# songrise/HyperNeRF-torch

Hardware: AMD Instinct MI355X
Metric: ray-samples/sec (fwd+bwd+Adam), whole job; per-GPU = value/n_gpus (higher is better)
Workload: dtype bf16; 1 GPU; NerfModel use_warp bendy_sheet nerf_embed+alpha_cond, 1024 rays x (64+64) samples per GPU, fwd+bwd+Adam; rays_per_gpu=1024, n_samples=64, n_importance=64, parallelism=dp1, hip_graph=True, wgrad_schedule=serial: one batched launch, optimizer_launch=hn_adam_step, ranks_seen_by_collective=1

## Files before the change

hypernerf-torch_amd/_lib.py:

```python
from __future__ import annotations

import ctypes as C
import os
import subprocess

import numpy as np
import torch

_HERE = os.path.dirname(os.path.abspath(__file__))
CSRC = os.path.join(_HERE, "csrc")
PRODUCT_LIB_PATH = os.path.join(CSRC, "libhn_hip.so")
LIB_PATH = os.environ.get("HN_LIB_PATH") or PRODUCT_LIB_PATH
SOURCES = ["hn_mlp.hip", "hn_render.hip", "hn_calib.hip", "hn_optim.hip"]
CSRC_HEADERS = ["hn_common.h", "hn_pack.h"]
HEADER = os.path.join(os.path.dirname(_HERE), "include", "hn_kernels.h")
BUILD_MACROS = ("HN_REDUCE_SPLIT", "HN_BF16_WAVES", "HN_PROF", "HN_CHUNK_UNITS", "HN_WGRAD_AUX", "HN_WGRAD_STAGES", "HN_WGRAD_MAXSLOT")

HN_MODE_F32, HN_MODE_BF16, HN_MODE_BF16_S8 = 0, 1, 2
BUILD_CONFIG_KEYS = ("WGRAD_STAGES", "WGRAD_MAXSLOT", "WGRAD_BIAS_MFMA", "CHUNK_UNITS", "WGRAD_BLOCK", "WSTREAM_ASYM",
                     "BF16_WAVES", "WGRAD_AUX")


def _read_build_config(path: str):
    import re
    try:
        with open(path, "rb") as f:
            blob = f.read()
    except OSError:
        return None
    m = re.search(rb"HN_BUILD_CONFIG:([0-9, ]+);", blob)
    if m is None:
        return None
    vals = [int(x) for x in m.group(1).decode().replace(" ", "").split(",")]
    return {k: v for k, v in zip(BUILD_CONFIG_KEYS, vals)}


BUILD_CONFIG = _read_build_config(LIB_PATH)
_cfg = BUILD_CONFIG or {}
WGRAD_STAGES = _cfg.get("WGRAD_STAGES", int(os.environ.get("HN_WGRAD_STAGES") or 2))
WGRAD_MAXSLOT = _cfg.get("WGRAD_MAXSLOT", int(os.environ.get("HN_WGRAD_MAXSLOT") or 8))
WGRAD_MAX_STAGE_KB = min(8 * WGRAD_MAXSLOT, 160 // WGRAD_STAGES)
HN_MAX_SRC, HN_MAX_DST, HN_MAX_SLOTS = 8, 4, 128
HN_OP_WORDS, HN_CHUNK_UNITS, HN_DSRC_COMPS = 8, _cfg.get("CHUNK_UNITS", int(os.environ.get("HN_CHUNK_UNITS", 32))), 32
HN_AUXG_MAX = 3
HN_MAX_COMPS = 32

HN_OP_LAYER, HN_OP_OUT, HN_OP_OUT_WIDE = 1, 4, 5
HN_ACT_NONE, HN_ACT_RELU, HN_ACT_LEAKY_RELU, HN_ACT_ELU, HN_ACT_SOFTPLUS = 0, 1, 2, 3, 4
HN_LAYER_NO_COMMIT, HN_LAYER_DIRECT = 1, 2
HN_BOP_LOAD, HN_BOP_LOAD_WIDE, HN_BOP_LAYER, HN_BOP_AUX = 1, 2, 3, 4
HN_FEAT_ZERO, HN_FEAT_ID, HN_FEAT_SIN, HN_FEAT_COS, HN_FEAT_SINP, HN_FEAT_ID_DIRECT = 0, 1, 2, 3, 4, 5


class HnSrc(C.Structure):
    _fields_ = [("ptr", C.c_void_p), ("ld", C.c_int32), ("per_ray", C.c_int32), ("gather_idx", C.c_void_p),
                ("gather_rows", C.c_int32), ("pad", C.c_int32)]


class HnDst(C.Structure):
    _fields_ = [("ptr", C.c_void_p), ("ld", C.c_int32), ("pad", C.c_int32)]


class HnSlot(C.Structure):
    _fields_ = [("off", C.c_uint64), ("nt", C.c_int32), ("pad", C.c_int32)]


class HnMlpArgs(C.Structure):
    _fields_ = [
        ("mode", C.c_int32), ("n_points", C.c_int32), ("samples_per_ray", C.c_int32), ("training", C.c_int32),
        ("n_ops", C.c_int32), ("n_chunks", C.c_int32), ("n_dsrc", C.c_int32), ("n_bias", C.c_int32),
        ("n_feat", C.c_int32), ("max_groups", C.c_int32),
        ("ops", C.c_void_p), ("wstream", C.c_void_p), ("bias", C.c_void_p), ("feat", C.c_void_p),
        ("stash", C.c_void_p), ("masks", C.c_void_p), ("dsrc", C.c_void_p),
        ("src", HnSrc * HN_MAX_SRC), ("dst", HnDst * HN_MAX_DST), ("slots", HnSlot * HN_MAX_SLOTS),
        ("prof", C.c_void_p), ("comps", C.c_void_p), ("n_comps", C.c_int32), ("embed_reg_mask", C.c_int32),
        ("embed_grad", C.c_void_p), ("embed_idx", C.c_void_p), ("embed_rows", C.c_int32), ("embed_dim", C.c_int32),
        ("embed_col", C.c_int8 * 32), ("n_trig_comps", C.c_int32), ("wide_ops", C.c_int32), ("dz_scale_log2", C.c_int32), ("trig_lo_planes", C.c_int32),
        ("timeline", C.c_void_p), ("embed_partial", C.c_void_p),
    ]


class HnDwBatch(C.Structure):
    _fields_ = [("jobs", C.c_void_p), ("stash", C.c_void_p), ("grads", C.c_void_p), ("n_jobs", C.c_int32),
                ("pad", C.c_int32), ("partials", C.c_void_p)]


HN_MAX_WGRAD_BATCH = 8
HN_MAX_DRAWS = 8


HN_MAX_PACK_JOBS = 8


class HnPackJob(C.Structure):
    _fields_ = [("units", C.c_void_p), ("ptrs", C.c_void_p), ("wstream", C.c_void_p), ("bias", C.c_void_p),
                ("bias_out", C.c_void_p), ("n_units", C.c_int32), ("n_bias", C.c_int32)]


class HnEmbedReduce(C.Structure):
    _fields_ = [("grad", C.c_void_p), ("rows", C.c_int32), ("dim", C.c_int32), ("col_mask", C.c_uint32), ("n_src", C.c_int32),
                ("partial", C.c_void_p * HN_MAX_WGRAD_BATCH), ("idx", C.c_void_p * HN_MAX_WGRAD_BATCH),
                ("n_blocks", C.c_int32 * HN_MAX_WGRAD_BATCH), ("samples_per_ray", C.c_int32 * HN_MAX_WGRAD_BATCH)]


class HnDraw(C.Structure):
    _fields_ = [("ptr", C.c_void_p), ("n", C.c_int64), ("kind", C.c_int32), ("pad", C.c_int32)]


class HnPrologue(C.Structure):
    _fields_ = [("t_rand_draw", C.c_int32), ("n_rays", C.c_int32), ("n", C.c_int32), ("ray_ld", C.c_int32),
                ("per_ray_bounds", C.c_int32), ("scale", C.c_float),
                ("origins", C.c_void_p), ("dirs", C.c_void_p), ("lower", C.c_void_p), ("upper", C.c_void_p),
                ("z_out", C.c_void_p), ("pts_out", C.c_void_p), ("ids_src", C.c_void_p), ("ids_dst", C.c_void_p),
                ("ids_ld", C.c_int32), ("n_ids", C.c_int32)]


class HnCompositeArgs(C.Structure):
    _fields_ = [
        ("variant", C.c_int32), ("n_rays", C.c_int32), ("n_samples", C.c_int32), ("white_bg", C.c_int32),
        ("sample_at_infinity", C.c_int32), ("warped_ld", C.c_int32), ("has_dust", C.c_int32), ("dust_threshold", C.c_float),
        ("rgb", C.c_void_p), ("raw", C.c_void_p), ("noise", C.c_void_p), ("z", C.c_void_p), ("dirs", C.c_void_p),
        ("ray_ld", C.c_int64), ("warped", C.c_void_p),
        ("out_rgb", C.c_void_p), ("out_depth", C.c_void_p), ("out_acc", C.c_void_p), ("out_weights", C.c_void_p),
        ("out_med_depth", C.c_void_p), ("out_med_points", C.c_void_p),
        ("g_rgb", C.c_void_p), ("g_depth", C.c_void_p), ("g_acc", C.c_void_p), ("g_weights", C.c_void_p),
        ("d_rgb", C.c_void_p), ("d_raw", C.c_void_p), ("keep", C.c_void_p),
        ("noise_scale", C.c_float), ("split", C.c_int32),
        ("perm", C.c_void_p), ("rgb1", C.c_void_p), ("raw1", C.c_void_p), ("warped1", C.c_void_p),
        ("d_rgb1", C.c_void_p), ("d_raw1", C.c_void_p), ("out_warped", C.c_void_p),
    ]


PACK_UNIT_DT = np.dtype([("w_id", "<i4"), ("ld", "<i4"), ("r0", "<i4"), ("c0", "<i4"), ("r_end", "<i4"),
                         ("c_end", "<i4"), ("k0", "<i4"), ("transposed", "<i4")])
PACK_BIAS_DT = np.dtype([("w_id", "<i4"), ("n", "<i4"), ("off", "<i4"), ("len", "<i4")])
FEAT_DT = np.dtype([("packed", "<i4"), ("freq", "<f4")])
DWJOB_DT = np.dtype([("z_off", "<u8"), ("x_off", "<u8"), ("z_nt", "<i4"), ("x_nt", "<i4"), ("z_t0", "<i4"),
                     ("x_t0", "<i4"), ("n_nt", "<i4"), ("n_kt", "<i4"), ("blk0", "<i4"), ("blk1", "<i4"),
                     ("w_off", "<i4"), ("ld", "<i4"), ("r0", "<i4"), ("c0", "<i4"), ("r_end", "<i4"),
                     ("c_end", "<i4"), ("b_off", "<i4"), ("pad", "<i4"), ("x2_off", "<u8"), ("x2_nt", "<i4"),
                     ("x2_t0", "<i4"), ("n_kt1", "<i4"), ("p_tile", "<i4")])
DWREDUCE_DT = np.dtype([("batch", "<i4"), ("w_off", "<i4"), ("ld", "<i4"), ("row0", "<i4"), ("col0", "<i4"),
                        ("r_end", "<i4"), ("c_end", "<i4"), ("first", "<i4"), ("count", "<i4")])

ADAM_RANGE_DT = np.dtype([("start", "<i8"), ("len", "<i4"), ("pad", "<i4")])


class HnAdamFuse(C.Structure):
    _fields_ = [("params", C.c_void_p), ("grads", C.c_void_p), ("exp_avg", C.c_void_p), ("exp_avg_sq", C.c_void_p),
                ("n", C.c_int64), ("hyper", C.c_void_p), ("step", C.c_void_p), ("rest", C.c_void_p),
                ("n_rest", C.c_int32), ("zero_grad", C.c_int32)]


EXPORTS = ["hn_version", "hn_abi_sizes", "hn_build_config", "hn_mlp_wgrad_reduce_adam", "hn_render_prologue", "hn_pack_units", "hn_pack_units_multi", "hn_mlp_forward", "hn_mlp_backward", "hn_mlp_wgrad",
           "hn_mlp_wgrad_batched", "hn_mlp_wgrad_batched_t", "hn_mlp_wgrad_reduce", "hn_mlp_workspace_bytes",
           "hn_sample_along_rays", "hn_sample_legacy", "hn_posenc", "hn_composite_forward", "hn_composite_backward", "hn_sample_pdf", "hn_sample_pdf_split", "hn_composite_sample_pdf",
           "hn_embed_gather", "hn_embed_backward", "hn_se3_apply_forward", "hn_se3_apply_backward", "hn_se3_warp_forward", "hn_se3_warp_backward", "hn_generate_rays", "hn_adam_step", "hn_sgd_step", "hn_radam_step",
           "hn_mse_loss_forward", "hn_mse_loss_backward", "hn_mse_loss_forward_grad", "hn_depth_index", "hn_random_fill",
           "hn_probe_mfma", "hn_calib_mfma", "hn_calib_stream", "hn_calib_stream_pattern", "hn_calib_ring"]

_lib = None


class HnError(RuntimeError):
    pass


def hipcc_path() -> str:
    for cand in (os.environ.get("HIPCC"), "/opt/rocm/bin/hipcc", "hipcc"):
        if cand and (os.path.isabs(cand) and os.path.exists(cand) or not os.path.isabs(cand)):
            return cand
    return "hipcc"


def needs_build() -> bool:
    if not os.path.exists(PRODUCT_LIB_PATH):
        return True
    t = os.path.getmtime(PRODUCT_LIB_PATH)
    deps = [os.path.join(CSRC, s) for s in SOURCES] + [os.path.join(CSRC, h) for h in CSRC_HEADERS] + [HEADER]
    return any(os.path.getmtime(d) > t for d in deps)


def build(force: bool = False, verbose: bool = False) -> str:
    if not force and not needs_build():
        return PRODUCT_LIB_PATH
    out = os.environ.get("HN_BUILD_OUT") or PRODUCT_LIB_PATH
    cmd = [hipcc_path(), "--offload-arch=gfx950", "-O3", "-std=c++17", "-ffp-contract=off", "-munsafe-fp-atomics", "-fPIC", "-shared",
           "-o", out] + [os.path.join(CSRC, s) for s in SOURCES]
    for macro in BUILD_MACROS:
        if os.environ.get(macro):
            cmd.insert(1, f"-D{macro}={os.environ[macro]}")
    res = subprocess.run(cmd, capture_output=True, text=True)
    if res.returncode != 0:
        raise HnError("hipcc failed:\n" + " ".join(cmd) + "\n" + res.stdout + res.stderr)
    if verbose:
        print(res.stdout + res.stderr)
    return out


def build_id() -> dict:
    import hashlib
    h = hashlib.sha256()
    for d in [os.path.join(CSRC, s) for s in SOURCES] + [os.path.join(CSRC, h) for h in CSRC_HEADERS] + [HEADER]:
        with open(d, "rb") as f:
            h.update(f.read())
    for macro in BUILD_MACROS:
        h.update(f"{macro}={os.environ.get(macro, '')};".encode())
    lib = None
    if os.path.exists(LIB_PATH):
        with open(LIB_PATH, "rb") as f:
            lib = hashlib.sha256(f.read()).hexdigest()[:16]
    ident = {"kernel_src_sha256": h.hexdigest()[:16], "lib_sha256": lib}
    if LIB_PATH != PRODUCT_LIB_PATH:
        ident["lib_path_override"] = LIB_PATH
        ident["kernel_src_sha256"] = "override:" + (lib or "?")
    if BUILD_CONFIG is not None:
        ident["build_config"] = dict(BUILD_CONFIG)
    return ident


def load():
    global _lib
    if _lib is not None:
        return _lib
    if not os.path.exists(LIB_PATH):
        raise HnError(
            f"{LIB_PATH} is missing: the HIP extension has not been built (run __graft_entry__.build()). "
            "hypernerf_torch_amd has no CPU fallback.")
    lib = C.CDLL(LIB_PATH)
    for name in EXPORTS:
        if not hasattr(lib, name):
            raise HnError(f"{LIB_PATH} does not export {name}")
        getattr(lib, name).restype = C.c_int
    buf = (C.c_int32 * len(BUILD_CONFIG_KEYS))()
    n_cfg = lib.hn_build_config(buf, len(BUILD_CONFIG_KEYS))
    now = {k: int(buf[i]) for i, k in enumerate(BUILD_CONFIG_KEYS[:n_cfg])}
    mine = {"WGRAD_STAGES": WGRAD_STAGES, "WGRAD_MAXSLOT": WGRAD_MAXSLOT, "CHUNK_UNITS": HN_CHUNK_UNITS}
    bad = {k: (v, now.get(k)) for k, v in mine.items() if now.get(k) != v}
    if bad:
        raise HnError(f"{LIB_PATH} was built with other tuning knobs than the host tables assume (mirror, library): {bad}; "
                      "re-import hypernerf_torch_amd after building, or unset the HN_* build variables")
    _lib = lib
    return lib


KERNEL_TIMES = None
_PENDING = []
PROF_BUFFER = None


def launch(name: str, *args, tag: str = ""):
    fn = getattr(load(), name)
    if KERNEL_TIMES is None:
        check(fn(*args), name + (f"[{tag}]" if tag else ""))
        return
    e0, e1 = torch.cuda.Event(enable_timing=True), torch.cuda.Event(enable_timing=True)
    e0.record()
    rc = fn(*args)
    e1.record()
    _PENDING.append((name + (f"[{tag}]" if tag else ""), e0, e1))
    check(rc, name)


TIMELINE = None
TIMELINE_TICK_S = 1e-8


def timeline_slot(name: str, device) -> int:
    if TIMELINE is None:
        return 0
    t = TIMELINE.get(name)
    if t is None:
        if torch.cuda.is_current_stream_capturing():
            raise HnError(f"kernel timeline: first launch of {name} inside a stream capture (run a warm-up step first)")
        t = TIMELINE[name] = torch.zeros(8, dtype=torch.int64, device=device)
    return t.data_ptr()


def timeline_reset():
    torch.cuda.synchronize()
    for t in (TIMELINE or {}).values():
        t.zero_()
    torch.cuda.synchronize()


def timeline_read() -> dict:
    torch.cuda.synchronize()
    out = {}
    for name, t in (TIMELINE or {}).items():
        v = t.cpu().tolist()
        out[name] = {"ms": v[4] * TIMELINE_TICK_S * 1e3, "runs": int(v[5]), "span_ms": (v[7] - v[6]) * TIMELINE_TICK_S * 1e3,
                     "first_start_tick": v[6], "last_end_tick": v[7]}
    return out


def collect_kernel_times():
    torch.cuda.synchronize()
    for name, e0, e1 in _PENDING:
        KERNEL_TIMES.setdefault(name, []).append(e0.elapsed_time(e1))
    _PENDING.clear()
    return KERNEL_TIMES


def check(rc: int, what: str):
    if rc != 0:
        kind = "argument error" if rc < 0 else "hipError_t"
        raise HnError(f"{what} failed: {kind} {rc}")


def stream_handle() -> C.c_void_p:
    return C.c_void_p(torch.cuda.current_stream().cuda_stream)


def require_gpu(*tensors):
    for t in tensors:
        if t is not None and not t.is_cuda:
            raise HnError("hypernerf_torch_amd runs on MI355X only: got a CPU tensor and there is no CPU fallback "
                          "(the CPU oracle lives in oracle/ and is test infrastructure)")

# ... 14 lines not shown
```

hypernerf-torch_amd/csrc/hn_mlp.hip:

```cpp
#include "hn_common.h"
#include <algorithm>
#include <type_traits>

#ifdef HN_PROF
#define HN_STAMP(code)                                                                          \
  do {                                                                                          \
    if (prof_on && prof_n < 2040) {                                                             \
      unsigned long long t__;                                                                   \
      __builtin_amdgcn_sched_barrier(0);                                                        \
      asm volatile("s_memtime %0\n\ts_waitcnt lgkmcnt(0)" : "=s"(t__)::"memory");               \
      __builtin_amdgcn_sched_barrier(0);                                                        \
      if (lane == 0) { prof_buf[2 * prof_n] = (code); prof_buf[2 * prof_n + 1] = (long long)t__; } \
      ++prof_n;                                                                                 \
    }                                                                                           \
  } while (0)
#else
#define HN_STAMP(code) do {} while (0)
#endif

template <int WAVES>
struct WStream {
  const char* g;
  char* lds;
  int ctr;
// ... 131 lines not shown
    va[j] = *reinterpret_cast<const float*>(srcv_r + (t[j][0] & 0xffffu));
    vb[j] = *reinterpret_cast<const float*>(srcv_r + (t[j][0] >> 16));
  }
  __builtin_amdgcn_sched_barrier(0);
#pragma unroll
  for (int j = 0; j < 4; ++j) {
    const float f = __uint_as_float(t[j][1]);
    const float big = __builtin_amdgcn_fractf(__fmul_rn(f, va[j]));
    const float sv = __builtin_amdgcn_sinf(__fadd_rn(big, __builtin_fmaf(f, vb[j], __uint_as_float(t[j][2]))));
    out[j] = hn_bfi(t[j][3], va[j], sv);
  }
}
HN_DEV void hn_feature_grads4(const HnDFeat* tp, const char* srcv_r, float* out) {
  u32x4 t[4];
#pragma unroll
  for (int j = 0; j < 4; ++j) t[j] = reinterpret_cast<const u32x4*>(tp)[j];
  __builtin_amdgcn_sched_barrier(0);
  float x[4];
#pragma unroll
  for (int j = 0; j < 4; ++j) x[j] = *reinterpret_cast<const float*>(srcv_r + t[j][0]);
  __builtin_amdgcn_sched_barrier(0);
#pragma unroll
  for (int j = 0; j < 4; ++j) {
    const float sc = __uint_as_float(t[j][1]);
    const float g = (sc * 6.283185307179586f) * hn_sin_rev(__builtin_fmaf(sc, x[j], __uint_as_float(t[j][2]) + 0.25f));
    out[j] = hn_bfi(t[j][3], 1.0f, g);
  }
}

template <bool BF16, bool DIRECT>
HN_DEV float hn_feature(const HnFeat e, const float* srcv, int r, const HnMlpArgs& a, int p, int ray) {
  const int kind = (e.packed >> 12) & 15;
  if constexpr (DIRECT) {
    if (kind == HN_FEAT_ID_DIRECT) return hn_direct_source(e, a, p, ray);
  }
  const float x = srcv[(e.packed & 255) * 32 + r];
  if constexpr (BF16) {
    const float ph = (kind == HN_FEAT_COS || kind == HN_FEAT_SINP) ? 0.25f : 0.0f;
    const float s = hn_sin_rev(__builtin_fmaf(e.freq * HN_INV_2PI, x, ph));
    return kind == HN_FEAT_ID ? x : (kind == HN_FEAT_ZERO ? 0.0f : s);
  } else {
    if (kind == HN_FEAT_ZERO) return 0.0f;
    if (kind == HN_FEAT_ID) return x;
    float arg = __fmul_rn(e.freq, x);
    if (kind == HN_FEAT_SINP) arg = __fadd_rn(arg, 0.5f * 3.1415926f);
    return kind == HN_FEAT_COS ? cosf(arg) : sinf(arg);
  }
}

template <bool BF16>
HN_DEV float hn_feature_grad(const HnFeat e, const float* srcv, int r) {
  const int kind = (e.packed >> 12) & 15;
  const float x = srcv[(e.packed & 255) * 32 + r];
  if constexpr (BF16) {
    const float ph = (kind == HN_FEAT_COS || kind == HN_FEAT_SINP) ? 0.5f : 0.25f;
    const float g = e.freq * hn_sin_rev(__builtin_fmaf(e.freq * HN_INV_2PI, x, ph));
    return (kind == HN_FEAT_ID || kind == HN_FEAT_ID_DIRECT) ? 1.0f : g;
  } else {
    if (kind == HN_FEAT_ID || kind == HN_FEAT_ID_DIRECT) return 1.0f;
    float arg = __fmul_rn(e.freq, x);
    if (kind == HN_FEAT_SINP) arg = __fadd_rn(arg, 0.5f * 3.1415926f);
    if (kind == HN_FEAT_COS) return -e.freq * sinf(arg);
    return e.freq * cosf(arg);
  }
}

template <bool DIRECT>
HN_DEV void hn_make_group(bf16x8* out, const HnFeat* ft, const HnDFeat* dft, const float* srcv, int lane,
                          const HnMlpArgs& a, int p, int ray) {
  const int h = lane >> 5, r = lane & 31;
  if constexpr (DIRECT) {
#pragma unroll
    for (int s = 0; s < 4; ++s) {
#pragma unroll
      for (int j = 0; j < 8; ++j)
        out[s][j] = (__bf16)hn_feature<true, true>(ft[16 * s + hn_pi16(h, j)], srcv, r, a, p, ray);
    }
  } else {
    const char* srcv_r = reinterpret_cast<const char*>(srcv) + 4 * r;
#pragma unroll
    for (int s = 0; s < 4; ++s) {
      float v[8];
      hn_features4(dft + 16 * s + 4 * h, srcv_r, v);
      hn_features4(dft + 16 * s + 8 + 4 * h, srcv_r, v + 4);
#pragma unroll
      for (int j = 0; j < 8; ++j) out[s][j] = (__bf16)v[j];
    }
  }
}
template <bool DIRECT>
HN_DEV void hn_make_group(float* out, const HnFeat* ft, const HnDFeat*, const float* srcv, int lane, const HnMlpArgs& a,
                          int p, int ray) {
  const int h = lane >> 5, r = lane & 31;
#pragma unroll
  for (int s = 0; s < 32; ++s) {
    out[s] = hn_feature<false, DIRECT>(ft[32 * (s >> 4) + hn_rho(s & 15, h)], srcv, r, a, p, ray);
    if ((s & 7) == 7) __builtin_amdgcn_sched_barrier(0);
  }
}

HN_DEV void hn_init_acc(f32x16& acc, const float* bias, int t, int h) {
  if (bias != nullptr) {
#pragma unroll
    for (int g = 0; g < 4; ++g) {
      const f32x4 b = *reinterpret_cast<const f32x4*>(bias + 32 * t + 8 * g + 4 * h);
      acc[4 * g] = b[0]; acc[4 * g + 1] = b[1]; acc[4 * g + 2] = b[2]; acc[4 * g + 3] = b[3];
    }
  } else {
#pragma unroll
    for (int i = 0; i < 16; ++i) acc[i] = 0.0f;
  }
}

constexpr int HN_PF = 3;
template <bool BF16, int K32>
HN_DEV void hn_gemm_blocks(f32x16& acc, const typename ModeT<BF16>::Frag* in, WStream<ModeT<BF16>::WAVES>& ws) {
  using M = ModeT<BF16>;
  const char* w = ws.take(K32 * M::UNITS32);
  if constexpr (BF16) {
    constexpr int N = 2 * K32;
    constexpr int D = N < HN_PF ? N : HN_PF;
    const char* wl = w + ws.lane * 16;
    bf16x8 q[D];
#pragma unroll
    for (int u = 0; u < D; ++u) q[u] = *reinterpret_cast<const bf16x8*>(wl + u * 1024);
#pragma unroll
    for (int u = 0; u < N; ++u) {
      acc = hn_mfma_bf16(q[u % D], in[u], acc);
      if (u + D < N) q[u % D] = *reinterpret_cast<const bf16x8*>(wl + (u + D) * 1024);
    }
    __builtin_amdgcn_sched_group_barrier(0x100, D, 0);
#pragma unroll
    for (int u = 0; u < N; ++u) {
      __builtin_amdgcn_sched_group_barrier(0x008, 1, 0);
      if (u + D < N) __builtin_amdgcn_sched_group_barrier(0x100, 1, 0);
    }
  } else {
#pragma unroll
    for (int k = 0; k < K32; ++k) hn_mma_block32(acc, w + k * M::UNITS32 * 1024, in + k * M::STEPS32, ws.lane);
  }
}
template <bool BF16>
HN_DEV void hn_gemm_k(f32x16& acc, const typename ModeT<BF16>::Frag* in, int K32, WStream<ModeT<BF16>::WAVES>& ws) {
  if (K32 == 8) hn_gemm_blocks<BF16, 8>(acc, in, ws);
  else if (K32 == 4) hn_gemm_blocks<BF16, 4>(acc, in, ws);
  else if (K32 == 2) hn_gemm_blocks<BF16, 2>(acc, in, ws);
  else if (K32 == 1) hn_gemm_blocks<BF16, 1>(acc, in, ws);
}

template <bool BF16, int S8 = 0>
HN_DEV char* hn_slot_base(const HnMlpArgs& a, int off_kib, int nt, int blk) {
  if (off_kib < 0) return nullptr;
  constexpr int TU = S8 ? 1 : ModeT<BF16>::TILE_UNITS;
  return reinterpret_cast<char*>(a.stash) + (size_t)(unsigned)off_kib * 1024 + (size_t)blk * nt * (TU * 1024);
}
HN_DEV uint32_t* hn_mask_base(const HnMlpArgs& a, int off256, int nt, int blk, int lane) {
  (void)lane;
  return a.masks + (size_t)(unsigned)off256 * 64 + (size_t)blk * nt * 64;
}
HN_DEV int hn_stash_slot(int r, int h, int u) { return 32 * h + (r ^ (4 * h + 8 * u)); }
HN_DEV int hn_stash8_slot(int r, int h) { return (r & 3) + 4 * h + 8 * ((r >> 2) & 1) + 16 * (r >> 3); }
template <int S8>
HN_DEV int hn_cvt2_f8(unsigned w, int old, bool hi) {
  const float lo_f = __uint_as_float(w << 16), hi_f = __uint_as_float(w & 0xffff0000u);
  if constexpr (S8 == 1) return hi ? __builtin_amdgcn_cvt_pk_fp8_f32(lo_f, hi_f, old, true)
                                   : __builtin_amdgcn_cvt_pk_fp8_f32(lo_f, hi_f, old, false);
  else return hi ? __builtin_amdgcn_cvt_pk_bf8_f32(lo_f, hi_f, old, true)
                 : __builtin_amdgcn_cvt_pk_bf8_f32(lo_f, hi_f, old, false);
}
template <int S8>
HN_DEV void hn_stash8_acc(const f32x16& a, char* slot_base, int t, int lane) {
  u32x4 o;
#pragma unroll
  for (int k = 0; k < 4; ++k) {
    int w = 0;
    if constexpr (S8 == 1) {
      w = __builtin_amdgcn_cvt_pk_fp8_f32(a[4 * k], a[4 * k + 1], w, false);
      w = __builtin_amdgcn_cvt_pk_fp8_f32(a[4 * k + 2], a[4 * k + 3], w, true);
    } else {
      w = __builtin_amdgcn_cvt_pk_bf8_f32(a[4 * k], a[4 * k + 1], w, false);
      w = __builtin_amdgcn_cvt_pk_bf8_f32(a[4 * k + 2], a[4 * k + 3], w, true);
    }
    o[k] = (unsigned)w;
  }
  char* dst8 = slot_base + (size_t)t * 1024 + hn_stash8_slot(lane & 31, lane >> 5) * 16;
  __builtin_nontemporal_store(o, reinterpret_cast<u32x4*>(dst8));
}
template <bool BF16, int S8 = 0>
HN_DEV void hn_stash(const typename ModeT<BF16>::Frag* fr, char* slot_base, int t, int lane) {
  using M = ModeT<BF16>;
  if constexpr (BF16 && S8 != 0) {
    const u32x4 f0 = *reinterpret_cast<const u32x4*>(&fr[0]), f1 = *reinterpret_cast<const u32x4*>(&fr[1]);
    u32x4 o;
#pragma unroll
    for (int k = 0; k < 2; ++k) {
      int lo = 0, hi = 0;
      lo = hn_cvt2_f8<S8>(f0[2 * k], lo, false);
      lo = hn_cvt2_f8<S8>(f0[2 * k + 1], lo, true);
      hi = hn_cvt2_f8<S8>(f1[2 * k], hi, false);
      hi = hn_cvt2_f8<S8>(f1[2 * k + 1], hi, true);
      o[k] = (unsigned)lo;
      o[2 + k] = (unsigned)hi;
    }
    char* dst8 = slot_base + (size_t)t * 1024 + hn_stash8_slot(lane & 31, lane >> 5) * 16;
    __builtin_nontemporal_store(o, reinterpret_cast<u32x4*>(dst8));
    return;
  }
  char* dst = slot_base + (size_t)t * (M::TILE_UNITS * 1024);
  if constexpr (BF16) {
    const int off0 = hn_stash_slot(lane & 31, lane >> 5, 0) * 16;
    __builtin_nontemporal_store(*reinterpret_cast<const u32x4*>(&fr[0]), reinterpret_cast<u32x4*>(dst + off0));
    __builtin_nontemporal_store(*reinterpret_cast<const u32x4*>(&fr[1]), reinterpret_cast<u32x4*>(dst + 1024 + (off0 ^ 128)));
  } else {
    const f32x16 z = hn_transpose_tile(fr, lane);
    hn_store_tile(z, dst, lane, (typename M::Frag*)nullptr);
  }
}

template <bool BF16>
HN_DEV unsigned hn_push_mask(unsigned bits, float x) {
  if constexpr (BF16) return __builtin_amdgcn_alignbit(bits, __float_as_uint(x), 31);
  return (bits << 1) | (x > 0.0f ? 0u : 1u);
}
HN_DEV int hn_keep_mask(unsigned nbits, int q, int i) { return (int)(nbits << (16 * q + i)) >> 31; }

template <bool BF16>
HN_DEV void hn_act_tile(f32x16& acc, int act, float p0, float p1, unsigned& bits) {
  if (act == HN_ACT_LEAKY_RELU) {
#pragma unroll 1
    for (int i = 0; i < 16; ++i) {
      bits = hn_push_mask<false>(bits, acc[i]);
      acc[i] = acc[i] > 0.0f ? acc[i] : p0 * acc[i];
    }
  } else if (act == HN_ACT_ELU) {
#pragma unroll 1
    for (int i = 0; i < 16; ++i) {
      const float z = acc[i];
      const float em1 = BF16 ? __expf(z) - 1.0f : expm1f(z);
      acc[i] = z > 0.0f ? z : p0 * em1;
    }
  } else if (act == HN_ACT_SOFTPLUS) {
    const float inv = 1.0f / p0;
#pragma unroll 1
    for (int i = 0; i < 16; ++i) {
      const float z = acc[i], u = z * p0;
      const float sp = BF16 ? __logf(1.0f + __expf(u)) : log1pf(expf(u));
      acc[i] = u > p1 ? z : (BF16 ? sp * inv : sp / p0);
    }
  }
}
template <bool BF16>
HN_DEV float hn_dact_y(int act, float y, float p0, float p1) {
  if (act == HN_ACT_ELU) return y > 0.0f ? 1.0f : y + p0;
  const float u = p0 * y;
  return u > p1 ? 1.0f : (BF16 ? 1.0f - __expf(-u) : -expm1f(-u));
}
template <bool BF16>
HN_DEV f32x16 hn_unstash(const char* slot_base, int t, int lane) {
  using M = ModeT<BF16>;
  const char* src = slot_base + (size_t)t * (M::TILE_UNITS * 1024);
  f32x16 y;
  if constexpr (BF16) {
    const int off0 = hn_stash_slot(lane & 31, lane >> 5, 0) * 16;
    const u32x4 f0 = *reinterpret_cast<const u32x4*>(src + off0);
    const u32x4 f1 = *reinterpret_cast<const u32x4*>(src + 1024 + (off0 ^ 128));
#pragma unroll
    for (int k = 0; k < 4; ++k) {
      y[2 * k] = __uint_as_float(f0[k] << 16);
      y[2 * k + 1] = __uint_as_float(f0[k] & 0xffff0000u);
      y[8 + 2 * k] = __uint_as_float(f1[k] << 16);
      y[8 + 2 * k + 1] = __uint_as_float(f1[k] & 0xffff0000u);
    }
  } else {
    float z[16];
#pragma unroll
    for (int g = 0; g < 4; ++g) {
      const f32x4 v = *reinterpret_cast<const f32x4*>(src + g * 1024 + lane * 16);
#pragma unroll
      for (int e = 0; e < 4; ++e) z[4 * g + e] = v[e];
    }
    y = hn_transpose_tile(z, lane);
  }
  return y;
}

typedef const __attribute__((address_space(4))) int* HnOpPtr;
HN_DEV HnOpPtr hn_op_words(const int* ops, int op) {
  return (HnOpPtr)(uintptr_t)(ops + (size_t)op * HN_OP_WORDS);
}
struct HnOpWords {
  int v[HN_OP_WORDS];
  HN_DEV int operator[](int i) const { return v[i]; }
};
HN_DEV HnOpWords hn_load_op(const int* ops, int op, int n_ops) {
  HnOpWords w;
  const HnOpPtr p = hn_op_words(ops, op < n_ops ? op : n_ops - 1);
#pragma unroll
  for (int i = 0; i < HN_OP_WORDS; ++i) w.v[i] = p[i];
  if (op >= n_ops) w.v[0] = -1;
  return w;
}


template <bool TRAIN, int NT, int S8>
HN_DEV void hn_epilogue_share(int k, int tp, f32x16& a, bf16x8* frag, unsigned& bits, char* out_base,
                              uint32_t* mask_base, int lane) {
  if (k < 8) {
#pragma unroll
    for (int e = 0; e < 2; ++e) {
      const int i = 2 * k + e;
      if (TRAIN) bits = hn_push_mask<true>(bits, a[i]);
      frag[i >> 3][i & 7] = (__bf16)__int_as_float(max(__float_as_int(a[i]), 0));
    }
  } else if (TRAIN && k == 8) {
    hn_stash<true, S8>(frag, out_base, tp, lane);
    if ((tp & 1) || tp == NT - 1) {
      mask_base[(tp >> 1) * 64 + lane] = (tp & 1) ? bits : bits << 16;
      bits = 0;
    }
  }
}

template <int K32, int NT, bool TRAIN, int S8>
HN_DEV void hn_layer_pipelined(bf16x8* cur, bf16x8* nxt, const float* bias, WStream<ModeT<true>::WAVES>& ws,
                               char* out_base, uint32_t* mask_base, int lane) {
  constexpr int N = 2 * K32;
  constexpr int D = 2;
  constexpr int SHARES = 9;
  constexpr int PER_SLOT = (SHARES + N - 1) / N;
  const int h = lane >> 5;
  f32x16 acc[2];
  unsigned bits = 0;
#pragma unroll
  for (int t = 0; t <= NT; ++t) {
    const char* wl = nullptr;
    if (t < NT) wl = ws.take(N) + lane * 16;
    const int tp = t - 1;
    bf16x8 q[D];
    if (t < NT) {
      hn_init_acc(acc[t & 1], bias, t, h);
#pragma unroll
      for (int u = 0; u < D; ++u) q[u] = *reinterpret_cast<const bf16x8*>(wl + u * 1024);
    }
    __builtin_amdgcn_sched_barrier(0);
#pragma unroll
    for (int u = 0; u < N; ++u) {
      if (t < NT) {
        acc[t & 1] = hn_mfma_bf16(q[u % D], cur[u], acc[t & 1]);
        if (u + D < N) q[u % D] = *reinterpret_cast<const bf16x8*>(wl + (u + D) * 1024);
      }
      if (t > 0) {
#pragma unroll
        for (int e = 0; e < PER_SLOT; ++e) {
          const int k = u * PER_SLOT + e;
          if (k < SHARES)
            hn_epilogue_share<TRAIN, NT, S8>(k, tp, acc[tp & 1], nxt + tp * 2, bits, out_base, mask_base, lane);
        }
      }
      __builtin_amdgcn_sched_barrier(0);
    }
  }
#pragma unroll
  for (int i = 0; i < NT * 2; ++i) cur[i] = nxt[i];
}

template <bool BF16, int AUXG, bool EXTRA, bool TRAIN, bool S8 = false>
__global__ __launch_bounds__(ModeT<BF16>::WAVES * 64, BF16 ? 2 : 1) void hn_mlp_fwd_kernel(const HnMlpArgs a) {
  using M = ModeT<BF16>;
  constexpr int SX = S8 ? 1 : 0;
  static_assert(!(S8 && (EXTRA || !TRAIN || !BF16)), "the 8-bit stash exists for the render-level bf16 training builds only");
  if constexpr (S8) asm volatile("s_setreg_imm32_b32 hwreg(HW_REG_MODE, 23, 1), 1");
  using Frag = typename M::Frag;
  extern __shared__ __attribute__((aligned(16))) char smem[];
  const int lane = threadIdx.x & 63;
  const int wave = __builtin_amdgcn_readfirstlane(threadIdx.x >> 6);
  const int r = lane & 31, h = lane >> 5;
  constexpr int PTS = M::WAVES * 32;
  const int ntiles = (a.n_points + PTS - 1) / PTS;
  hn_timeline_begin(a.timeline);
#ifdef HN_PROF
  long long* prof_buf = reinterpret_cast<long long*>(a.prof);
  const bool prof_on = prof_buf != nullptr && blockIdx.x == 0 && wave == 0;
  int prof_n = 0;
#endif

  WStream<M::WAVES> ws;
  ws.g = reinterpret_cast<const char*>(a.wstream);
  ws.lds = smem;
  ws.nchunks = a.n_chunks;
  ws.wave = wave;
  ws.lane = lane;

  Frag cur[8 * M::STEPS32];
  Frag nxt[8 * M::STEPS32];

  float* bias_lds = reinterpret_cast<float*>(smem + 2 * HN_CHUNK_UNITS * 1024);
  HnFeat* feat_lds = reinterpret_cast<HnFeat*>(bias_lds + ((a.n_bias + 3) & ~3));
  HnDFeat* dfeat_lds = reinterpret_cast<HnDFeat*>(feat_lds + ((a.n_feat + 1) & ~1));
  const int n_trig = BF16 ? a.n_trig_comps : 0;
  const bool with_lo = a.trig_lo_planes != 0;
  const int n_planes = BF16 ? a.n_comps + n_trig + (with_lo ? n_trig : 1) : a.n_comps;
  float* srcv = reinterpret_cast<float*>(BF16 ? reinterpret_cast<char*>(dfeat_lds + a.n_feat)
                                              : reinterpret_cast<char*>(dfeat_lds)) + wave * (n_planes * 32);
  float* rev = BF16 ? srcv + a.n_comps * 32 : nullptr;
  for (int i = threadIdx.x; i < a.n_bias; i += blockDim.x) bias_lds[i] = a.bias[i];
  for (int i = threadIdx.x; i < a.n_feat; i += blockDim.x) {
    const HnFeat e = a.feat[i];
    feat_lds[i] = e;
    if constexpr (BF16) dfeat_lds[i] = hn_derive_feat_fwd(e, a.n_comps, n_trig, with_lo);
  }
  __syncthreads();

  for (int tile = blockIdx.x; tile < ntiles; tile += gridDim.x) {
    const int blk = tile * M::WAVES + wave;
    const int p0 = blk * 32 + r;
    const bool valid = p0 < a.n_points;
    const int p = valid ? p0 : a.n_points - 1;
    const int ray = p / a.samples_per_ray;
    const bool wave_valid = blk * 32 < a.n_points;
    hn_stage_sources(srcv, a, p, ray, lane, rev, n_trig, with_lo);
    ws.start();

    HnOpWords w_next = hn_load_op(a.ops, 0, a.n_ops);
    for (int op = 0; op < a.n_ops; ++op) {
      const HnOpWords w = w_next;
      w_next = hn_load_op(a.ops, op + 1, a.n_ops);
      const int code = w[0];
      if (code == HN_OP_LAYER) {
        HN_STAMP(100 + op);
        const int K32 = w[1] & 255, nG = (w[1] >> 8) & 255, NT = (w[1] >> 16) & 255;
        const int act = (w[1] >> 24) & 15, flags = (w[1] >> 28) & 15;
        const float* bias = bias_lds + w[2];
        const bool do_mask = TRAIN && w[4] >= 0 && wave_valid && act != HN_ACT_SOFTPLUS;
        const bool do_stash = TRAIN && w[5] >= 0 && wave_valid;
        char* out_base = do_stash ? hn_slot_base<BF16, SX>(a, w[5], NT, blk) : nullptr;
        char* aux_base = (TRAIN && wave_valid) ? hn_slot_base<BF16, SX>(a, w[6], 2 * nG, blk) : nullptr;
        uint32_t* mask_base = do_mask ? hn_mask_base(a, w[4], (NT + 1) >> 1, blk, lane) : nullptr;
        const bool has_out = w_next[0] == HN_OP_OUT;
        const HnOpWords out_w = w_next;
        Frag aux[AUXG * 2 * M::STEPS32];
#pragma unroll
        for (int g = 0; g < AUXG; ++g) {
          if (g < nG) {
            if (EXTRA && (flags & HN_LAYER_DIRECT))
              hn_make_group<true>(aux + g * 2 * M::STEPS32, feat_lds + w[3] + 64 * g, dfeat_lds + w[3] + 64 * g, srcv,
                                  lane, a, p, ray);
            else
              hn_make_group<false>(aux + g * 2 * M::STEPS32, feat_lds + w[3] + 64 * g, dfeat_lds + w[3] + 64 * g, srcv,
                                   lane, a, p, ray);
            if (aux_base != nullptr) {
              hn_stash<BF16, SX>(aux + g * 2 * M::STEPS32, aux_base, 2 * g, lane);
              hn_stash<BF16, SX>(aux + (g * 2 + 1) * M::STEPS32, aux_base, 2 * g + 1, lane);
            }
          }
        }
        unsigned bits = 0;
        HN_STAMP(1);
        if constexpr (BF16) {
          const bool plain = nG == 0 && act == HN_ACT_RELU && !(flags & HN_LAYER_NO_COMMIT) && !has_out &&
                             wave_valid && do_stash == do_mask;
          if (plain && K32 == 4 && NT == 4) {
            if (do_stash) hn_layer_pipelined<4, 4, true, SX>(cur, nxt, bias, ws, out_base, mask_base, lane);
            else hn_layer_pipelined<4, 4, false, SX>(cur, nxt, bias, ws, out_base, mask_base, lane);
            continue;
          }
        }
#pragma unroll
        for (int t = 0; t < 8; ++t) {
          if (t < NT) {
            f32x16 acc;
            hn_init_acc(acc, bias, t, h);
            hn_gemm_k<BF16>(acc, cur, K32, ws);
#pragma unroll
            for (int g = 0; g < AUXG; ++g)
              if (g < nG) hn_gemm_blocks<BF16, 2>(acc, aux + g * 2 * M::STEPS32, ws);
            HN_STAMP(2);
            if (act == HN_ACT_RELU) {
#pragma unroll
              for (int i = 0; i < 16; ++i) {
                bits = hn_push_mask<BF16>(bits, acc[i]);
                acc[i] = __int_as_float(max(__float_as_int(acc[i]), 0));
              }
            } else if (act != HN_ACT_NONE) {
              hn_act_tile<BF16>(acc, act, __int_as_float(w[7]), __int_as_float(w[4]), bits);
            }
            if (has_out && t == 0 && h == 0 && valid) {
              const HnDst d = a.dst[out_w[1]];
              const int n = out_w[3];
#pragma unroll
              for (int i = 0; i < 4; ++i) {
                if (i < n) {
                  float y = acc[i];
                  if (out_w[4] == 1) y = 1.0f / (1.0f + expf(-y));
                  if (out_w[5] >= 0) {
                    const HnSrc sr = a.src[out_w[5]];
                    y = __fadd_rn(sr.ptr[(size_t)(sr.per_ray ? ray : p) * sr.ld + out_w[6] + i], y);
                  }
                  d.ptr[(size_t)p * d.ld + out_w[2] + i] = y;
                }
              }
            }
            if (has_out && t == 0 && h == 0 && out_w[7] > 0) {
              const int n = out_w[3];
#pragma unroll
              for (int i = 0; i < 4; ++i) {
                if (i < n) {
                  float y = acc[i];
                  if (out_w[4] == 1) y = 1.0f / (1.0f + expf(-y));
                  if (out_w[5] >= 0) {
                    const HnSrc sr = a.src[out_w[5]];
                    y = __fadd_rn(sr.ptr[(size_t)(sr.per_ray ? ray : p) * sr.ld + out_w[6] + i], y);
                  }
                  const int ci = out_w[7] - 1 + i;
                  srcv[ci * 32 + r] = y;
                  if (BF16 && ci < n_trig) {
                    float hi, lo;
                    hn_rev_split(y, hi, lo);
                    rev[ci * 32 + r] = hi;
                    if (with_lo) rev[(n_trig + ci) * 32 + r] = lo;
                  }
                }
              }
            }
            hn_acc_to_frags(acc, nxt + t * M::STEPS32);
#ifdef HN_PROF
            if (prof_on) {
              float x__ = acc[15];
              asm volatile("v_mov_b32 %0, %0" : "+v"(x__)::"memory");
            }
#endif
            HN_STAMP(3);
            if ((t & 1) || t == NT - 1) {
              if (do_mask) mask_base[(t >> 1) * 64 + lane] = (t & 1) ? bits : bits << 16;
              bits = 0;
            }
            if (do_stash) {
              if constexpr (SX != 0) hn_stash8_acc<SX>(acc, out_base, t, lane);
              else hn_stash<BF16, SX>(nxt + t * M::STEPS32, out_base, t, lane);
            }
            HN_STAMP(4);
          }
        }
        if (!(flags & HN_LAYER_NO_COMMIT)) {
#pragma unroll
          for (int t = 0; t < 8; ++t)
            if (t < NT)
#pragma unroll
              for (int s = 0; s < M::STEPS32; ++s) cur[t * M::STEPS32 + s] = nxt[t * M::STEPS32 + s];
        }
      } else if (code == HN_OP_OUT) {
      } else if (EXTRA && code == HN_OP_OUT_WIDE) {
        const int n = w[3], NT = w[4];
        if (valid) {
          const HnDst d = a.dst[w[1]];
#pragma unroll
          for (int t = 0; t < 8; ++t)
            if (t < NT) {
              if constexpr (BF16) {
#pragma unroll
                for (int s = 0; s < 2; ++s)
#pragma unroll
                  for (int j = 0; j < 8; ++j) {
                    const int row = 32 * t + 16 * s + hn_pi16(h, j);
                    if (row < n) d.ptr[(size_t)p * d.ld + w[2] + row] = (float)cur[2 * t + s][j];
                  }
              } else {
#pragma unroll
                for (int q = 0; q < 16; ++q) {
                  const int row = 32 * t + hn_rho(q, h);
                  if (row < n) d.ptr[(size_t)p * d.ld + w[2] + row] = cur[16 * t + q];
                }
              }
            }
        }
      }
    }
  }
  hn_timeline_end(a.timeline);
}

HN_DEV bool hn_prefetch_masks(const HnMlpArgs& a, const HnOpWords& wn, int blk, int lane, bool wave_valid,
                              unsigned* out) {
  if (wn[0] != HN_BOP_LAYER || wn[4] < 0) return false;
  const int NT = (wn[1] >> 16) & 255;
  const uint32_t* mb = hn_mask_base(a, wn[4], (NT + 1) >> 1, blk, lane);
#pragma unroll
  for (int dd = 0; dd < 4; ++dd)
    out[dd] = (2 * dd < NT) ? (wave_valid ? mb[dd * 64 + lane] : 0xffffffffu) : 0u;
  return true;
}

template <bool BF16, bool WIDE, bool S8 = false>
__global__ __launch_bounds__(ModeT<BF16>::WAVES * 64, BF16 ? 2 : 1) void hn_mlp_bwd_kernel(const HnMlpArgs a) {
  using M = ModeT<BF16>;
  constexpr int SZ = S8 ? 2 : 0;
  static_assert(!(S8 && WIDE) && !(S8 && !BF16), "the 8-bit stash exists for the render-level bf16 builds only");
  if constexpr (S8) asm volatile("s_setreg_imm32_b32 hwreg(HW_REG_MODE, 23, 1), 1");
  const float dz_scale = S8 ? ldexpf(1.0f, a.dz_scale_log2) : 1.0f;
  const float dz_unscale = S8 ? ldexpf(1.0f, -a.dz_scale_log2) : 1.0f;
  using Frag = typename M::Frag;
  extern __shared__ __attribute__((aligned(16))) char smem[];
  const int lane = threadIdx.x & 63;
  const int wave = __builtin_amdgcn_readfirstlane(threadIdx.x >> 6);
  const int r = lane & 31, h = lane >> 5;
  constexpr int PTS = M::WAVES * 32;
  const int ntiles = (a.n_points + PTS - 1) / PTS;
  HnFeat* feat_lds = reinterpret_cast<HnFeat*>(smem + 2 * HN_CHUNK_UNITS * 1024);
  HnDFeat* dfeat_lds = reinterpret_cast<HnDFeat*>(feat_lds + ((a.n_feat + 1) & ~1));
  float* srcv = reinterpret_cast<float*>(BF16 ? reinterpret_cast<char*>(dfeat_lds + a.n_feat)
                                              : reinterpret_cast<char*>(dfeat_lds)) + wave * (a.n_comps * 32);
  hn_timeline_begin(a.timeline);
#ifdef HN_PROF
  long long* prof_buf = reinterpret_cast<long long*>(a.prof);
  const bool prof_on = prof_buf != nullptr && blockIdx.x == 0 && wave == 0;
  int prof_n = 0;
#endif
  for (int i = threadIdx.x; i < a.n_feat; i += blockDim.x) {
    const HnFeat e = a.feat[i];
    feat_lds[i] = e;
    if constexpr (BF16) dfeat_lds[i] = hn_derive_feat(e);
  }
  __syncthreads();

  WStream<M::WAVES> ws;
  ws.g = reinterpret_cast<const char*>(a.wstream);
  ws.lds = smem;
  ws.nchunks = a.n_chunks;
  ws.wave = wave;
  ws.lane = lane;

  Frag cur[8 * M::STEPS32];
  Frag nxt[8 * M::STEPS32];
  Frag cur2[M::STEPS32];

  for (int tile = blockIdx.x; tile < ntiles; tile += gridDim.x) {
    const int blk = tile * M::WAVES + wave;
    const int p0 = blk * 32 + r;
    const bool valid = p0 < a.n_points;
    const int p = valid ? p0 : a.n_points - 1;
    const int ray = p / a.samples_per_ray;
    const bool wave_valid = blk * 32 < a.n_points;
    f32x16 dacc;
    hn_init_acc(dacc, nullptr, 0, h);
    hn_stage_sources(srcv, a, p, ray, lane);
    ws.start();

    HnOpWords w_next = hn_load_op(a.ops, 0, a.n_ops);
    unsigned mnext[4] = {0u, 0u, 0u, 0u};
    bool mnext_ready = false;
    for (int op = 0; op < a.n_ops; ++op) {
      const HnOpWords w = w_next;
      w_next = hn_load_op(a.ops, op + 1, a.n_ops);
      const int code = w[0];
      HN_STAMP(100 * code + op);
      if (code != HN_BOP_LAYER && code != HN_BOP_AUX) mnext_ready = false;
      if (code == HN_BOP_LOAD) {
        const int n = w[3] & 255;
        const bool to2 = (w[3] >> 8) & 1;
        float d[4] = {0.f, 0.f, 0.f, 0.f};
        if ((w[3] >> 9) & 1) {
          const int q = (w[3] >> 10) & 3;
#pragma unroll
          for (int i = 0; i < 4; ++i)
            d[i] = q == 0 ? dacc[i] : (q == 1 ? dacc[4 + i] : (q == 2 ? dacc[8 + i] : dacc[12 + i]));
        }
        if (h == 0 && valid) {
          const HnSrc s = a.src[w[1] < 0 ? 0 : w[1]];
#pragma unroll
          for (int i = 0; i < 4; ++i)
            if (i < n) {
              float g = (w[1] >= 0 && s.ptr != nullptr) ? s.ptr[(size_t)p * s.ld + w[2] + i] : 0.0f;
              if constexpr (S8) g *= dz_scale;
              if ((w[3] >> 9) & 1) g += d[i];
              if (w[4] == 1) {
                const HnSrc ys = a.src[w[5]];
                const float y = ys.ptr[(size_t)p * ys.ld + w[6] + i];
                g = g * y * (1.0f - y);
              }
              d[i] = g;
            } else {
              d[i] = 0.0f;
            }
        } else {
#pragma unroll
          for (int i = 0; i < 4; ++i) d[i] = 0.0f;
        }
        Frag tmp[M::STEPS32];
        hn_zero_frags(tmp, M::STEPS32);
        if constexpr (BF16) {
#pragma unroll
          for (int i = 0; i < 4; ++i) tmp[0][i] = (__bf16)d[i];
        } else {
#pragma unroll
          for (int i = 0; i < 4; ++i) tmp[i] = d[i];
        }
        if (a.training && w[7] >= 0 && wave_valid) hn_stash<BF16, SZ>(tmp, hn_slot_base<BF16, SZ>(a, w[7], 1, blk), 0, lane);
#pragma unroll
        for (int s = 0; s < M::STEPS32; ++s) {
          if (to2) cur2[s] = tmp[s];
          else cur[s] = tmp[s];
        }
      } else if (WIDE && code == HN_BOP_LOAD_WIDE) {
        const int n = w[3] & 0xffff, NT = w[4], dact = (w[3] >> 16) & 15;
        const HnSrc s = a.src[w[1]];
        unsigned nbits = 0xffffffffu;
        char* dz_base = (a.training && wave_valid) ? hn_slot_base<BF16>(a, w[7], NT, blk) : nullptr;
        const bool has_mask = w[5] >= 0 && dact != HN_ACT_SOFTPLUS;
        const bool from_y = (dact == HN_ACT_ELU || dact == HN_ACT_SOFTPLUS) && wave_valid;
        const char* y_base = from_y ? hn_slot_base<BF16>(a, w[7], NT, blk) : nullptr;
#pragma unroll
        for (int t = 0; t < 8; ++t) {
          if (t < NT) {
            if (has_mask && !(t & 1)) {
              nbits = wave_valid ? ~hn_mask_base(a, w[5], (NT + 1) >> 1, blk, lane)[(t >> 1) * 64 + lane] : 0u;
            }
            f32x16 v;
            if (dact == 0) {
#pragma unroll
              for (int i = 0; i < 16; ++i) {
                const int row = 32 * t + hn_rho(i, h);
                const bool keep = hn_keep_mask(nbits, t & 1, i) != 0;
                v[i] = (valid && keep && row < n) ? s.ptr[(size_t)p * s.ld + w[2] + row] : 0.0f;
              }
            } else {
              const float p0 = __int_as_float(w[6]), p1 = __int_as_float(w[5]);
              f32x16 y = {0};
              if (y_base != nullptr) y = hn_unstash<BF16>(y_base, t, lane);
#pragma unroll
              for (int i = 0; i < 16; ++i) {
                const int row = 32 * t + hn_rho(i, h);
                const float g = (valid && row < n) ? s.ptr[(size_t)p * s.ld + w[2] + row] : 0.0f;
                float d = 1.0f;
                if (dact == HN_ACT_LEAKY_RELU) d = hn_keep_mask(nbits, t & 1, i) != 0 ? 1.0f : p0;
                else d = hn_dact_y<BF16>(dact, y[i], p0, p1);
                v[i] = g * d;
              }
            }
            hn_acc_to_frags(v, cur + t * M::STEPS32);
            if (dz_base != nullptr) hn_stash<BF16>(cur + t * M::STEPS32, dz_base, t, lane);
          }
        }
      } else if (code == HN_BOP_LAYER) {
        const int K32 = w[1] & 255, K32b = (w[1] >> 8) & 255, NT = (w[1] >> 16) & 255;
        const bool has_mask = w[4] >= 0;
        const bool do_stash = a.training && w[5] >= 0 && wave_valid;
        char* dz_base = do_stash ? hn_slot_base<BF16, SZ>(a, w[5], NT, blk) : nullptr;
        const int dact = w[2];
        const char* y_base = (!S8 && (dact == HN_ACT_ELU || dact == HN_ACT_SOFTPLUS) && wave_valid)
                                 ? hn_slot_base<BF16>(a, w[6], NT, blk) : nullptr;
        unsigned nbits = 0xffffffffu;
        unsigned mbits[4] = {0xffffffffu, 0xffffffffu, 0xffffffffu, 0xffffffffu};
        if (has_mask) {
          if (mnext_ready) {
#pragma unroll
            for (int dd = 0; dd < 4; ++dd) mbits[dd] = ~mnext[dd];
          } else {
            const uint32_t* mb = hn_mask_base(a, w[4], (NT + 1) >> 1, blk, lane);
#pragma unroll
            for (int dd = 0; dd < 4; ++dd)
              if (2 * dd < NT)
                mbits[dd] = wave_valid ? ~mb[dd * 64 + lane] : 0u;
          }
        }
        mnext_ready = false;
#pragma unroll
        for (int t = 0; t < 8; ++t) {
          if (t < NT) {
// ... 1199 lines not shown
```

Before: 82.65 million ray-samples/s.

## Extend pipelined forward MLP layer to aux-input groups and more layer shapes

Generalizes the software-pipelined forward layer, which overlaps the next tile's MFMA chain with the previous tile's ReLU/stash epilogue, so it also covers layers that consume auxiliary input groups and additional K/NT shapes. A shape dispatcher instantiates the pipeline for a fixed set of (K32, nG, NT) combinations, and a build macro can disable it. The aim is to hide epilogue latency on more of the MLP layers. In exchange, the pipelined path is now restricted to the non-S8, non-EXTRA builds, which drops it from the 8-bit stash path that previously used it, and the many template instantiations add code size and register pressure.

```diff
diff --git a/hypernerf-torch_amd/_lib.py b/hypernerf-torch_amd/_lib.py
--- a/hypernerf-torch_amd/_lib.py
+++ b/hypernerf-torch_amd/_lib.py
@@ -14,7 +14,7 @@
 SOURCES = ["hn_mlp.hip", "hn_render.hip", "hn_calib.hip", "hn_optim.hip"]
 CSRC_HEADERS = ["hn_common.h", "hn_pack.h"]
 HEADER = os.path.join(os.path.dirname(_HERE), "include", "hn_kernels.h")
-BUILD_MACROS = ("HN_REDUCE_SPLIT", "HN_BF16_WAVES", "HN_PROF", "HN_CHUNK_UNITS", "HN_WGRAD_AUX", "HN_WGRAD_STAGES", "HN_WGRAD_MAXSLOT")
+BUILD_MACROS = ("HN_REDUCE_SPLIT", "HN_BF16_WAVES", "HN_PROF", "HN_FWD_PIPELINE", "HN_CHUNK_UNITS", "HN_WGRAD_AUX", "HN_WGRAD_STAGES", "HN_WGRAD_MAXSLOT")
 
 HN_MODE_F32, HN_MODE_BF16, HN_MODE_BF16_S8 = 0, 1, 2
 BUILD_CONFIG_KEYS = ("WGRAD_STAGES", "WGRAD_MAXSLOT", "WGRAD_BIAS_MFMA", "CHUNK_UNITS", "WGRAD_BLOCK", "WSTREAM_ASYM",
diff --git a/hypernerf-torch_amd/csrc/hn_mlp.hip b/hypernerf-torch_amd/csrc/hn_mlp.hip
--- a/hypernerf-torch_amd/csrc/hn_mlp.hip
+++ b/hypernerf-torch_amd/csrc/hn_mlp.hip
@@ -457,6 +457,9 @@
 }
 
 
+#ifndef HN_FWD_PIPELINE
+#define HN_FWD_PIPELINE 1
+#endif
 template <bool TRAIN, int NT, int S8>
 HN_DEV void hn_epilogue_share(int k, int tp, f32x16& a, bf16x8* frag, unsigned& bits, char* out_base,
                               uint32_t* mask_base, int lane) {
@@ -476,47 +479,83 @@
   }
 }
 
-template <int K32, int NT, bool TRAIN, int S8>
-HN_DEV void hn_layer_pipelined(bf16x8* cur, bf16x8* nxt, const float* bias, WStream<ModeT<true>::WAVES>& ws,
-                               char* out_base, uint32_t* mask_base, int lane) {
-  constexpr int N = 2 * K32;
+template <int K32, int NG, int NT, bool TRAIN, int S8>
+HN_DEV void hn_layer_pipelined(bf16x8* cur, bf16x8* nxt, const bf16x8* aux, const float* bias,
+                               WStream<ModeT<true>::WAVES>& ws, char* out_base, uint32_t* mask_base, int lane) {
+  constexpr int NSEG = (K32 > 0 ? 1 : 0) + NG;
+  constexpr int S = 2 * K32 + 4 * NG;
   constexpr int D = 2;
   constexpr int SHARES = 9;
-  constexpr int PER_SLOT = (SHARES + N - 1) / N;
+  constexpr int PER_SLOT = (SHARES + S - 1) / S;
+  static_assert(NSEG > 0 && 2 * K32 <= 16, "a pipelined layer has products, at most 8 blocks of cur");
   const int h = lane >> 5;
   f32x16 acc[2];
   unsigned bits = 0;
 #pragma unroll
   for (int t = 0; t <= NT; ++t) {
-    const char* wl = nullptr;
-    if (t < NT) wl = ws.take(N) + lane * 16;
     const int tp = t - 1;
-    bf16x8 q[D];
-    if (t < NT) {
-      hn_init_acc(acc[t & 1], bias, t, h);
-#pragma unroll
-      for (int u = 0; u < D; ++u) q[u] = *reinterpret_cast<const bf16x8*>(wl + u * 1024);
-    }
-    __builtin_amdgcn_sched_barrier(0);
-#pragma unroll
-    for (int u = 0; u < N; ++u) {
+#pragma unroll
+    for (int seg = 0; seg < NSEG; ++seg) {
+      const bool is_cur = K32 > 0 && seg == 0;
+      const int n = is_cur ? 2 * K32 : 4;
+      const int g = seg - (K32 > 0 ? 1 : 0);
+      const int off = is_cur ? 0 : 2 * K32 + 4 * g;
+      const bf16x8* in = is_cur ? cur : aux + 4 * g;
+      const char* wl = nullptr;
+      if (t < NT) wl = ws.take(n) + lane * 16;
+      bf16x8 q[D];
       if (t < NT) {
-        acc[t & 1] = hn_mfma_bf16(q[u % D], cur[u], acc[t & 1]);
-        if (u + D < N) q[u % D] = *reinterpret_cast<const bf16x8*>(wl + (u + D) * 1024);
-      }
-      if (t > 0) {
-#pragma unroll
-        for (int e = 0; e < PER_SLOT; ++e) {
-          const int k = u * PER_SLOT + e;
-          if (k < SHARES)
-            hn_epilogue_share<TRAIN, NT, S8>(k, tp, acc[tp & 1], nxt + tp * 2, bits, out_base, mask_base, lane);
-        }
+        if (seg == 0) hn_init_acc(acc[t & 1], bias, t, h);
+#pragma unroll
+        for (int u = 0; u < D; ++u) q[u] = *reinterpret_cast<const bf16x8*>(wl + u * 1024);
       }
       __builtin_amdgcn_sched_barrier(0);
+#pragma unroll
+      for (int u = 0; u < 16; ++u) {
+        if (u < n) {
+          if (t < NT) {
+            acc[t & 1] = hn_mfma_bf16(q[u % D], in[u], acc[t & 1]);
+            if (u + D < n) q[u % D] = *reinterpret_cast<const bf16x8*>(wl + (u + D) * 1024);
+          }
+          if (t > 0) {
+#pragma unroll
+            for (int e = 0; e < PER_SLOT; ++e) {
+              const int k = (off + u) * PER_SLOT + e;
+              if (k < SHARES)
+                hn_epilogue_share<TRAIN, NT, S8>(k, tp, acc[tp & 1], nxt + tp * 2, bits, out_base, mask_base, lane);
+            }
+          }
+          __builtin_amdgcn_sched_barrier(0);
+        }
+      }
     }
   }
 #pragma unroll
   for (int i = 0; i < NT * 2; ++i) cur[i] = nxt[i];
+}
+
+template <bool STASH, int AUXG>
+HN_DEV bool hn_layer_pipelined_shape(int K32, int nG, int NT, bf16x8* cur, bf16x8* nxt, const bf16x8* aux,
+                                     const float* bias, WStream<ModeT<true>::WAVES>& ws, char* out_base,
+                                     uint32_t* mask_base, int lane) {
+#define HN_PIPE(k, g, n)                                                                            \
+  if (K32 == (k) && nG == (g) && NT == (n)) {                                                       \
+    hn_layer_pipelined<k, g, n, STASH, 0>(cur, nxt, aux, bias, ws, out_base, mask_base, lane);     \
+    return true;                                                                                    \
+  }
+  HN_PIPE(4, 0, 4)
+  HN_PIPE(2, 0, 2)
+  if constexpr (AUXG >= 1) {
+    HN_PIPE(0, 1, 2)
+    HN_PIPE(2, 1, 2)
+    HN_PIPE(4, 1, 4)
+  }
+  if constexpr (AUXG >= 2) {
+    HN_PIPE(0, 2, 4)
+    HN_PIPE(4, 2, 4)
+  }
+#undef HN_PIPE
+  return false;
 }
 
 template <bool BF16, int AUXG, bool EXTRA, bool TRAIN, bool S8 = false>
@@ -612,12 +651,12 @@
         unsigned bits = 0;
         HN_STAMP(1);
         if constexpr (BF16) {
-          const bool plain = nG == 0 && act == HN_ACT_RELU && !(flags & HN_LAYER_NO_COMMIT) && !has_out &&
-                             wave_valid && do_stash == do_mask;
-          if (plain && K32 == 4 && NT == 4) {
-            if (do_stash) hn_layer_pipelined<4, 4, true, SX>(cur, nxt, bias, ws, out_base, mask_base, lane);
-            else hn_layer_pipelined<4, 4, false, SX>(cur, nxt, bias, ws, out_base, mask_base, lane);
-            continue;
+          if constexpr (SX == 0 && !EXTRA) {
+            const bool plain = act == HN_ACT_RELU && !(flags & HN_LAYER_NO_COMMIT) && !has_out && wave_valid &&
+                               do_stash == TRAIN && do_mask == TRAIN;
+            if (HN_FWD_PIPELINE && plain &&
+                hn_layer_pipelined_shape<TRAIN, AUXG>(K32, nG, NT, cur, nxt, aux, bias, ws, out_base, mask_base, lane))
+              continue;
           }
         }
 #pragma unroll
```

Measured after the change: 82.66 million ray-samples/s (median of 5 runs). About the same (+0.0%).
